# Kainmueller-Lab/PatchPerPix

Hardware: AMD Instinct MI355X
Metric: Mvoxels/sec assembled (vote_instances) (higher is better)
Workload: dtype f16 in, f32 accumulate

## Files before the change

include/ppp_mi355x.h:

```cpp
#ifndef PPP_MI355X_H
#define PPP_MI355X_H

#include <stddef.h>
#include <stdint.h>

#ifdef __cplusplus
extern "C" {
#endif

#define PPP_ABI_VERSION 5

enum ppp_error {
    PPP_OK = 0,
    PPP_ERR_INVALID_ARG = -1,
    PPP_ERR_NO_DEVICE = -2,
    PPP_ERR_HIP = -3,
    PPP_ERR_UNSUPPORTED = -4,
    PPP_ERR_WORKSPACE = -5
};

enum ppp_dtype { PPP_F32 = 0, PPP_F16 = 1, PPP_BF16 = 2 };

enum ppp_bg_rule { PPP_BG_INV_TH = 0, PPP_BG_HALF_TH = 1, PPP_BG_LESS_THAN_TH = 2 };
enum ppp_value_rule { PPP_VAL_COUNT = 0, PPP_VAL_PROB_PRODUCT = 1, PPP_VAL_NORM_PROB_PRODUCT = 2 };
// ... 210 lines not shown
                   const ppp_params *p, void *stream);

int64_t ppp_thin_shard_workspace_bytes(const ppp_params *p);
int ppp_thin_open(const uint8_t *d_mask, const int64_t *d_lin, const int32_t *d_index, int64_t n, int32_t *d_state,
                  int32_t *d_count, int32_t *d_cleared, void *d_work, const ppp_params *p, void *stream);
int ppp_thin_step(int32_t what, const uint32_t *d_bits, int32_t *d_state, int32_t *d_count, int32_t *d_cleared,
                  void *d_work, int32_t global_z, const ppp_params *p, void *stream);
int ppp_thin_alive(void *d_work, const ppp_params *p, void *stream, int32_t *alive);
int ppp_thin_close(uint8_t *d_mask, void *d_work, const ppp_params *p, void *stream);
int ppp_thin_zone(int32_t import, void *d_work, int32_t z_lo, int32_t z_hi, int32_t own_lo, int32_t own_hi,
                  int64_t *d_key, uint8_t *d_mask, uint8_t *d_clean, const ppp_params *p, void *stream);

int ppp_patch_pairs_count(const int32_t *d_sorted_zyx, int64_t n, int32_t max_ps_dist,
                          int64_t *d_counts, const ppp_params *p, void *stream);
int ppp_patch_pairs_fill(const int32_t *d_sorted_zyx, int64_t n, int32_t max_ps_dist,
                         const int64_t *d_offsets, int64_t n_pair_rows, int32_t include_single,
                         uint32_t *d_rows, const ppp_params *p, void *stream);
int ppp_patch_pairs_count_subset(const int32_t *d_sorted_zyx, int64_t n, int32_t max_ps_dist,
                                 const int64_t *d_subset, int64_t m, int64_t *d_counts,
                                 const ppp_params *p, void *stream);
int ppp_patch_pairs_fill_subset(const int32_t *d_sorted_zyx, int64_t n, int32_t max_ps_dist,
                                const int64_t *d_subset, int64_t m, const int64_t *d_local_offsets,
                                const int64_t *d_global_offsets, int64_t n_local_rows,
                                int64_t n_rows_total, int32_t include_single, uint32_t *d_rows,
                                int64_t *d_row_ids, const ppp_params *p, void *stream);
int ppp_patch_pairs_count_slices(const int32_t *d_sorted_zyx, int64_t n, int32_t max_ps_dist,
                                 int64_t *d_counts, const ppp_params *p, void *stream);
int ppp_patch_pairs_fill_slices(const int32_t *d_sorted_zyx, int64_t n, int32_t max_ps_dist,
                                const int64_t *d_offsets, int64_t n_pair_rows, int32_t include_single,
                                uint32_t *d_rows, const ppp_params *p, void *stream);
int ppp_patch_graph_slices(const void *d_pred, int pred_dtype, const float *d_cons,
                           const uint32_t *d_pairs, const uint32_t *d_order, uint64_t n_pairs,
                           float *d_aff, const ppp_params *p, void *stream);
int ppp_patch_graph_lcg_slices(const void *d_pred, int pred_dtype, const uint32_t *d_pairs,
                               const uint32_t *d_order, const int64_t *d_lcg_pos, int64_t n_lcg,
                               const int64_t *d_drop_off, uint64_t *d_drops, const ppp_params *p,
                               void *stream);
int ppp_patch_graph_by_patch_lcg_slices(const void *d_pred, int pred_dtype, const float *d_cons_vm,
                                        const uint32_t *d_pairs, const uint32_t *d_order,
                                        const int64_t *d_group_start, const int64_t *d_chunk_offsets,
                                        int32_t n_groups, int64_t n_blocks, int32_t chunk, float *d_aff,
                                        const int64_t *d_drop_off, const uint64_t *d_drops,
                                        const ppp_params *p, void *stream);
int ppp_thin_cover_slices(const uint8_t *d_mask, const uint32_t *d_bits, const int64_t *d_lin, int64_t n,
                          uint8_t *d_keep, void *d_work, const int64_t *h_slice_interior,
                          const ppp_params *p, void *stream, int32_t *rounds);
int ppp_label_slice_renumber(const uint32_t *d_nodes, uint64_t n_nodes, int32_t *d_labels,
                             int32_t *d_slice_min, int32_t *d_slice_max, const ppp_params *p, void *stream);

int ppp_pair_sort_keys(const uint32_t *d_rows, uint64_t n_rows, int64_t *d_keys,
                       const ppp_params *p, void *stream);
#define PPP_PAIR_KEY_FAR 0x7FFFFFFFFFFFFFFFll
int ppp_pair_group_keys(const uint32_t *d_rows, uint64_t n_rows, int64_t *d_keys,
                        const ppp_params *p, void *stream);

int64_t ppp_host_rank_order(const float *h_score, const uint8_t *h_foreground, const int32_t *vol,
                            const int32_t *patchshape, int64_t *out_lin);
int64_t ppp_host_cover_pass(uint8_t *h_mask_running, const uint8_t *h_overlap, const int32_t *vol,
                            const int32_t *patchshape, const int64_t *ranked_lin,
                            const float *ranked_score, const uint32_t *bits, int64_t n,
                            int32_t pix_th, double score_threshold, uint8_t *selected,
                            int64_t *remaining, int32_t *stopped);
int64_t ppp_host_cover_pass_marked(uint8_t *h_mask_running, const uint8_t *h_overlap, const int32_t *vol,
                                   const int32_t *patchshape, const int64_t *ranked_lin,
                                   const float *ranked_score, const uint32_t *bits, int64_t n,
                                   int32_t pix_th, double score_threshold, uint8_t *selected,
                                   int64_t *remaining, int32_t *stopped, uint8_t *h_marked);
int64_t ppp_host_thin_cover(const uint8_t *h_mask, const int32_t *vol, const int32_t *patchshape,
                            const int64_t *sel_lin, const uint32_t *bits, int64_t n,
                            uint8_t *keep);

int64_t ppp_host_skeletonize_3d(const uint8_t *h_mask, const int32_t *vol, uint8_t *h_out);
int64_t ppp_host_skel_rule_mismatches(uint32_t first, uint32_t count);
int64_t ppp_host_patch_pairs(const int32_t *sel_zyx, int64_t n, const int32_t *patchshape,
                             int32_t max_ps_dist, int32_t include_single, int32_t *sorted_zyx,
                             uint32_t *pairs);

int64_t ppp_host_mws(const uint32_t *pairs, const float *aff, int64_t n_rows, const int32_t *vol,
                     int32_t *out_nodes, int32_t *out_labels, int64_t cap, int64_t *n_labels);

int64_t ppp_host_mws_sorted(const int32_t *eu, const int32_t *ev, int64_t n_edges, int64_t n_nodes,
                            int32_t *labels);

int64_t ppp_host_pack_channels(int64_t n_labels, const int64_t *sizes, const uint64_t *pairs, int64_t n_pairs,
                               int64_t min_voxels, int32_t *chan_out, int32_t *n_channels_out);

int64_t ppp_rank_order_workspace_bytes(const ppp_params *p);
int ppp_rank_order(const float *d_score, const uint8_t *d_foreground, int64_t *d_lin,
                   float *d_rank_score, int64_t *count, void *d_work, const ppp_params *p,
                   void *stream);
int64_t ppp_mws_edges_workspace_bytes(int64_t n_rows, int64_t n_nodes, const ppp_params *p);
int ppp_mws_edges(const uint32_t *d_pairs, const float *d_aff, int64_t n_rows, const uint32_t *d_nodes,
                  int64_t n_nodes, int32_t *d_eu, int32_t *d_ev, int64_t *n_edges, void *d_work,
                  const ppp_params *p, void *stream);

int64_t ppp_post_compact_ids_workspace_bytes(int64_t n, uint32_t max_id);
int ppp_post_compact_ids(uint32_t *d_ids, int64_t n, uint32_t max_id, int64_t compsize, int32_t relabel,
                         uint32_t start, int64_t *n_kept, void *d_work, void *stream);
int64_t ppp_post_dilate_workspace_bytes(int32_t Z, int32_t Y, int32_t X);
int ppp_post_dilate(const uint32_t *d_in, uint32_t *d_out, int32_t Z, int32_t Y, int32_t X, int32_t *rounds,
                    void *d_work, void *stream);
int64_t ppp_post_clean_mask_workspace_bytes(int32_t Z, int32_t Y, int32_t X);
int ppp_post_clean_mask(const uint8_t *d_mask, uint8_t *d_out, int32_t Z, int32_t Y, int32_t X, uint32_t structure,
                        int64_t size, int64_t *n_found, int64_t *n_kept, void *d_work, void *stream);

int64_t ppp_post_edt_sq_workspace_bytes(int32_t Z, int32_t Y, int32_t X);
int ppp_post_edt_sq(const uint8_t *d_feature, uint32_t *d_out, int32_t Z, int32_t Y, int32_t X, uint32_t cap,
                    void *d_work, void *stream);
int64_t ppp_post_fg_filter_workspace_bytes(int32_t Z, int32_t Y, int32_t X);
int ppp_post_fg_filter(const uint8_t *d_mask, uint8_t *d_fg , uint32_t *d_inst ,
                       int32_t Z, int32_t Y, int32_t X, int64_t compsize, uint32_t min_d2,
                       int64_t *stats , void *d_work, void *stream);

int32_t ppp_eval_patch_thresholds_per_pass(void);
int32_t ppp_eval_patch_max_thresholds(void);
int64_t ppp_eval_patch_workspace_bytes(const int32_t *vol , int32_t tz);
int ppp_eval_patch(const void *d_pred, int pred_dtype, int32_t C, const int32_t *d_labels, int32_t L,
                   const int32_t *vol , const int32_t *patch , int32_t z0, int32_t tz,
                   const float *thresholds , int32_t T, int64_t *d_counts ,
                   int32_t *d_inter, int32_t *d_union , void *d_work, void *stream);

int64_t ppp_skeletonize_3d_workspace_bytes(int32_t Z, int32_t Y, int32_t X);
int ppp_skeletonize_3d(const uint8_t *d_mask, uint8_t *d_out, int32_t Z, int32_t Y, int32_t X,
                       int64_t *n_kept, int32_t *stats ,
                       void *d_work, void *stream);

int64_t ppp_skeletonize_labels_workspace_bytes(int32_t Z, int32_t Y, int32_t X);
int ppp_skeletonize_labels(const uint32_t *d_labels, uint32_t *d_out, int32_t Z, int32_t Y, int32_t X,
                           int64_t *n_kept, int32_t *stats ,
                           void *d_work, void *stream);

int32_t ppp_label_overlap_table_entries(void);
void ppp_label_overlap_last_stats(int64_t *stats );
uint32_t ppp_label_overlap_slot(uint32_t a, uint32_t b);
int64_t ppp_label_overlap_workspace_bytes(int32_t La, int32_t Lb, int32_t Z, int32_t Y, int32_t X);
int ppp_label_overlap(const uint32_t *d_a, int32_t La, const uint32_t *d_b, int32_t Lb,
                      int32_t Z, int32_t Y, int32_t X,
                      uint32_t *d_rows , int64_t *d_counts , int64_t cap,
                      int64_t *n_rows , void *d_work, void *stream);

int ppp_patch_mosaic(const void *d_pred, int pred_dtype, int32_t C, const uint8_t *d_selected, int32_t S,
                     void *d_out, int32_t tz, int32_t Y, int32_t X, const int32_t *patch , void *stream);

int ppp_gt_affs_dense_plan(int32_t B, int32_t L, const int32_t *vol , int32_t E, const int32_t *halo ,
                           const int32_t *box , int out_dtype, int32_t single, int32_t *plan );
int ppp_gt_affs_dense(const int32_t *d_labels, int32_t B, int32_t L, const int32_t *vol ,
                      const int32_t *d_nhood, int32_t E, const int32_t *halo ,
                      const int32_t *box , void *d_out, int out_dtype, int32_t single, void *stream);
int ppp_gt_affs_samples(const int32_t *d_labels, int32_t B, int32_t L, const int32_t *vol ,
                        const int32_t *d_samples , int64_t N, const int32_t *d_nhood, int32_t E,
                        const int32_t *ps , const int32_t *ctr , void *d_out, int out_dtype,
                        void *stream);

int64_t ppp_patch_loss_workspace_bytes(int32_t B, int32_t L, const int32_t *vol , int32_t E,
                                       const int32_t *halo , const int32_t *box ,
                                       int dtype, int64_t N );
int ppp_patch_loss_dense_fwd(const void *d_logits, int dtype, const int32_t *d_labels, int32_t B, int32_t L,
                             const int32_t *vol , const int32_t *d_nhood, int32_t E, const int32_t *halo ,
                             const int32_t *box , const float *d_weight , double num_channels,
                             float *d_loss , double *d_state , int64_t *d_counts ,
                             void *d_work, void *stream);
int ppp_patch_loss_dense_bwd(const void *d_logits, int dtype, const int32_t *d_labels, int32_t B, int32_t L,
                             const int32_t *vol , const int32_t *d_nhood, int32_t E, const int32_t *halo ,
                             const int32_t *box , const float *d_weight ,
                             const double *d_state , const float *d_grad_out , void *d_grad,
                             void *stream);
// ... 45 lines not shown
```

patchperpix_amd/backend.py:

```python
import ctypes
import os

import numpy as np

from . import build as _build

F32, F16, BF16 = 0, 1, 2
BG_INV_TH, BG_HALF_TH, BG_LESS_THAN_TH = 0, 1, 2
VAL_COUNT, VAL_PROB_PRODUCT, VAL_NORM_PROB_PRODUCT = 0, 1, 2
CONS_COMPACT, CONS_REFERENCE, CONS_VOXEL_MAJOR = 0, 1, 2
ABI_VERSION = 5
NONE_KEY = 0xFFFFFFFF
NONE_KEY64 = 1 << 62
PAIR_KEY_FAR = 0x7FFFFFFFFFFFFFFF


class Box(ctypes.Structure):
    _fields_ = [(n, ctypes.c_int32) for n in ("z0", "y0", "x0", "z1", "y1", "x1")]

    def shape(self):
        return (self.z1 - self.z0, self.y1 - self.y0, self.x1 - self.x0)


class Params(ctypes.Structure):
# ... 116 lines not shown
    "ppp_patch_graph_by_patch_bits": (ctypes.c_int, [ctypes.c_void_p, ctypes.c_int, ctypes.c_void_p,
                                                     ctypes.c_void_p, ctypes.c_void_p, ctypes.c_void_p,
                                                     ctypes.c_void_p, ctypes.c_int32, ctypes.c_int64,
                                                     ctypes.c_int32, ctypes.c_void_p, ctypes.c_void_p,
                                                     ctypes.c_void_p, ctypes.c_void_p, ctypes.c_int64,
                                                     ctypes.c_void_p, ctypes.c_int32,
                                                     ctypes.POINTER(Params), ctypes.c_void_p]),
    "ppp_label_workspace_bytes": (ctypes.c_size_t, [ctypes.POINTER(Params)]),
    "ppp_label_components": (ctypes.c_int, [ctypes.c_void_p, ctypes.c_void_p, ctypes.c_uint64,
                                            ctypes.c_void_p, ctypes.c_uint64, ctypes.c_void_p,
                                            ctypes.c_void_p, ctypes.POINTER(Params),
                                            ctypes.c_void_p]),
    "ppp_label_begin": (ctypes.c_int, [ctypes.c_void_p, ctypes.c_uint64, ctypes.c_void_p,
                                       ctypes.POINTER(Params), ctypes.c_void_p]),
    "ppp_label_add": (ctypes.c_int, [ctypes.c_void_p, ctypes.c_void_p, ctypes.c_void_p,
                                     ctypes.c_int64, ctypes.c_uint64, ctypes.c_void_p,
                                     ctypes.POINTER(Params), ctypes.c_void_p]),
    "ppp_label_union_edges": (ctypes.c_int, [ctypes.c_void_p, ctypes.c_void_p, ctypes.c_uint64,
                                             ctypes.c_void_p, ctypes.POINTER(Params),
                                             ctypes.c_void_p]),
    "ppp_label_finish": (ctypes.c_int, [ctypes.c_void_p, ctypes.c_uint64, ctypes.c_void_p,
                                        ctypes.c_void_p, ctypes.POINTER(Params), ctypes.c_void_p]),
    "ppp_patch_pairs_count_subset": (ctypes.c_int, [ctypes.c_void_p, ctypes.c_int64, ctypes.c_int32,
                                                    ctypes.c_void_p, ctypes.c_int64, ctypes.c_void_p,
                                                    ctypes.POINTER(Params), ctypes.c_void_p]),
    "ppp_patch_pairs_fill_subset": (ctypes.c_int, [ctypes.c_void_p, ctypes.c_int64, ctypes.c_int32,
                                                   ctypes.c_void_p, ctypes.c_int64, ctypes.c_void_p,
                                                   ctypes.c_void_p, ctypes.c_int64, ctypes.c_int64,
                                                   ctypes.c_int32, ctypes.c_void_p, ctypes.c_void_p,
                                                   ctypes.POINTER(Params), ctypes.c_void_p]),
    "ppp_patch_pairs_count": (ctypes.c_int, [ctypes.c_void_p, ctypes.c_int64, ctypes.c_int32,
                                             ctypes.c_void_p, ctypes.POINTER(Params),
                                             ctypes.c_void_p]),
    "ppp_patch_pairs_fill": (ctypes.c_int, [ctypes.c_void_p, ctypes.c_int64, ctypes.c_int32,
                                            ctypes.c_void_p, ctypes.c_int64, ctypes.c_int32,
                                            ctypes.c_void_p, ctypes.POINTER(Params),
                                            ctypes.c_void_p]),
    "ppp_pair_sort_keys": (ctypes.c_int, [ctypes.c_void_p, ctypes.c_uint64, ctypes.c_void_p,
                                          ctypes.POINTER(Params), ctypes.c_void_p]),
    "ppp_paint_instances": (ctypes.c_int, [ctypes.c_void_p, ctypes.c_int, ctypes.c_void_p,
                                           ctypes.c_void_p, ctypes.c_uint64, ctypes.c_void_p,
                                           ctypes.POINTER(Params), ctypes.c_void_p]),
    "ppp_cons_to_reference": (ctypes.c_int, [ctypes.c_void_p, ctypes.c_void_p,
                                             ctypes.POINTER(Params), ctypes.c_void_p]),
    "ppp_cons_to_voxel_major": (ctypes.c_int, [ctypes.c_void_p, ctypes.c_void_p,
                                               ctypes.POINTER(Params), ctypes.c_void_p]),
    "ppp_patch_bits": (ctypes.c_int, [ctypes.c_void_p, ctypes.c_int, ctypes.c_void_p,
                                      ctypes.c_uint64, ctypes.c_double, ctypes.c_void_p,
                                      ctypes.POINTER(Params), ctypes.c_void_p]),
    "ppp_patch_bits_volume": (ctypes.c_int, [ctypes.c_void_p, ctypes.c_int, ctypes.c_double,
                                             ctypes.c_void_p, ctypes.POINTER(Params), ctypes.c_void_p]),
    "ppp_pair_group_keys": (ctypes.c_int, [ctypes.c_void_p, ctypes.c_uint64, ctypes.c_void_p,
                                           ctypes.POINTER(Params), ctypes.c_void_p]),
    "ppp_patch_graph_by_patch_chunk": (ctypes.c_int32, [ctypes.POINTER(Params)]),
    "ppp_cover_workspace_bytes": (ctypes.c_int64, [ctypes.c_int64, ctypes.POINTER(Params)]),
    "ppp_cover_pass": (ctypes.c_int, [ctypes.c_void_p, ctypes.c_void_p, ctypes.c_void_p,
                                      ctypes.c_int64, ctypes.c_int32, ctypes.c_void_p,
                                      ctypes.c_void_p, ctypes.c_void_p, ctypes.POINTER(Params),
                                      ctypes.c_void_p, ctypes.POINTER(ctypes.c_int32)]),
    "ppp_cover_pass_voxel_bits": (ctypes.c_int, [ctypes.c_void_p, ctypes.c_void_p, ctypes.c_int64,
                                                 ctypes.c_void_p, ctypes.c_int64, ctypes.c_int32,
                                                 ctypes.c_void_p, ctypes.c_void_p, ctypes.c_void_p,
                                                 ctypes.POINTER(Params), ctypes.c_void_p,
                                                 ctypes.POINTER(ctypes.c_int32)]),
    "ppp_cover_pass_marked": (ctypes.c_int, [ctypes.c_void_p, ctypes.c_void_p, ctypes.c_void_p,
                                             ctypes.c_int64, ctypes.c_int32, ctypes.c_void_p,
                                             ctypes.c_void_p, ctypes.c_void_p, ctypes.c_void_p,
                                             ctypes.POINTER(Params), ctypes.c_void_p,
                                             ctypes.POINTER(ctypes.c_int32)]),
    "ppp_cover_pass_marked_voxel_bits": (ctypes.c_int, [ctypes.c_void_p, ctypes.c_void_p, ctypes.c_int64,
                                                        ctypes.c_void_p, ctypes.c_int64, ctypes.c_int32,
                                                        ctypes.c_void_p, ctypes.c_void_p, ctypes.c_void_p,
                                                        ctypes.c_void_p, ctypes.POINTER(Params),
                                                        ctypes.c_void_p, ctypes.POINTER(ctypes.c_int32)]),
    "ppp_cover_mark_bits_bytes": (ctypes.c_int64, [ctypes.POINTER(Params)]),
    "ppp_cover_marks_from_selected": (ctypes.c_int, [ctypes.c_void_p, ctypes.c_void_p, ctypes.c_int64,
                                                     ctypes.c_void_p, ctypes.POINTER(Params),
                                                     ctypes.c_void_p]),
    "ppp_mask_dilate_workspace_bytes": (ctypes.c_int64, [ctypes.POINTER(Params)]),
    "ppp_mask_dilate": (ctypes.c_int, [ctypes.c_void_p, ctypes.c_void_p, ctypes.c_int32, ctypes.c_int32,
                                       ctypes.c_void_p, ctypes.POINTER(Params), ctypes.c_void_p]),
    "ppp_host_mws_sorted": (ctypes.c_int64, [ctypes.c_void_p, ctypes.c_void_p, ctypes.c_int64,
                                             ctypes.c_int64, ctypes.c_void_p]),
    "ppp_rank_order_workspace_bytes": (ctypes.c_int64, [ctypes.POINTER(Params)]),
    "ppp_rank_order": (ctypes.c_int, [ctypes.c_void_p, ctypes.c_void_p, ctypes.c_void_p,
                                      ctypes.c_void_p, ctypes.POINTER(ctypes.c_int64),
                                      ctypes.c_void_p, ctypes.POINTER(Params), ctypes.c_void_p]),
    "ppp_mws_edges_workspace_bytes": (ctypes.c_int64, [ctypes.c_int64, ctypes.c_int64,
                                                       ctypes.POINTER(Params)]),
    "ppp_mws_edges": (ctypes.c_int, [ctypes.c_void_p, ctypes.c_void_p, ctypes.c_int64,
                                     ctypes.c_void_p, ctypes.c_int64, ctypes.c_void_p,
                                     ctypes.c_void_p, ctypes.POINTER(ctypes.c_int64),
                                     ctypes.c_void_p, ctypes.POINTER(Params), ctypes.c_void_p]),
    "ppp_thin_workspace_bytes": (ctypes.c_int64, [ctypes.c_int64, ctypes.POINTER(Params)]),
    "ppp_thin_cover": (ctypes.c_int, [ctypes.c_void_p, ctypes.c_void_p, ctypes.c_void_p,
                                      ctypes.c_int64, ctypes.c_void_p, ctypes.c_void_p,
                                      ctypes.POINTER(Params), ctypes.c_void_p,
                                      ctypes.POINTER(ctypes.c_int32)]),
    "ppp_cover_open": (ctypes.c_int, [ctypes.c_void_p, ctypes.c_void_p, ctypes.c_void_p,
                                      ctypes.c_int64, ctypes.c_void_p, ctypes.c_void_p,
                                      ctypes.c_void_p, ctypes.POINTER(Params), ctypes.c_void_p]),
    "ppp_cover_step": (ctypes.c_int, [ctypes.c_int32, ctypes.c_void_p, ctypes.c_int32,
                                      ctypes.c_void_p, ctypes.c_void_p, ctypes.c_void_p,
                                      ctypes.c_int32, ctypes.POINTER(Params), ctypes.c_void_p]),
    "ppp_cover_alive": (ctypes.c_int, [ctypes.c_void_p, ctypes.POINTER(Params), ctypes.c_void_p,
                                       ctypes.POINTER(ctypes.c_int32)]),
    "ppp_cover_close": (ctypes.c_int, [ctypes.c_void_p, ctypes.c_void_p, ctypes.POINTER(Params),
                                       ctypes.c_void_p]),
    "ppp_cover_zone": (ctypes.c_int, [ctypes.c_int32, ctypes.c_void_p, ctypes.c_int32,
                                      ctypes.c_int32, ctypes.c_int32, ctypes.c_int32,
                                      ctypes.c_void_p, ctypes.c_void_p, ctypes.c_void_p,
                                      ctypes.POINTER(Params), ctypes.c_void_p]),
    "ppp_thin_shard_workspace_bytes": (ctypes.c_int64, [ctypes.POINTER(Params)]),
    "ppp_thin_open": (ctypes.c_int, [ctypes.c_void_p, ctypes.c_void_p, ctypes.c_void_p, ctypes.c_int64,
                                     ctypes.c_void_p, ctypes.c_void_p, ctypes.c_void_p, ctypes.c_void_p,
                                     ctypes.POINTER(Params), ctypes.c_void_p]),
    "ppp_thin_step": (ctypes.c_int, [ctypes.c_int32, ctypes.c_void_p, ctypes.c_void_p, ctypes.c_void_p,
                                     ctypes.c_void_p, ctypes.c_void_p, ctypes.c_int32, ctypes.POINTER(Params),
                                     ctypes.c_void_p]),
    "ppp_thin_alive": (ctypes.c_int, [ctypes.c_void_p, ctypes.POINTER(Params), ctypes.c_void_p,
                                      ctypes.POINTER(ctypes.c_int32)]),
    "ppp_thin_close": (ctypes.c_int, [ctypes.c_void_p, ctypes.c_void_p, ctypes.POINTER(Params), ctypes.c_void_p]),
    "ppp_thin_zone": (ctypes.c_int, [ctypes.c_int32, ctypes.c_void_p, ctypes.c_int32, ctypes.c_int32,
                                     ctypes.c_int32, ctypes.c_int32, ctypes.c_void_p, ctypes.c_void_p,
                                     ctypes.c_void_p, ctypes.POINTER(Params), ctypes.c_void_p]),
    "ppp_synth_pred": (ctypes.c_int, [ctypes.c_void_p, ctypes.c_void_p, ctypes.c_int,
                                      ctypes.c_uint32, ctypes.c_float, ctypes.c_float,
                                      ctypes.c_float, ctypes.c_uint64, ctypes.POINTER(Params),
                                      ctypes.c_void_p]),
    "ppp_synth_pred_box": (ctypes.c_int, [ctypes.c_void_p, ctypes.c_void_p, ctypes.c_void_p, ctypes.c_int,
                                          ctypes.c_uint32, ctypes.c_float, ctypes.c_float, ctypes.c_float,
                                          ctypes.c_void_p, ctypes.POINTER(Params), ctypes.c_void_p]),
    "ppp_decode_tail": (ctypes.c_int, [ctypes.c_void_p, ctypes.c_int64, ctypes.c_int32, ctypes.c_int32,
                                       ctypes.c_void_p, ctypes.c_float, ctypes.c_void_p, ctypes.c_float,
                                       ctypes.c_void_p, ctypes.c_float, ctypes.c_void_p, ctypes.c_void_p,
                                       ctypes.c_int, ctypes.POINTER(Params), ctypes.c_void_p]),
    "ppp_decode_tail_rows": (ctypes.c_int, [ctypes.c_void_p, ctypes.c_int64, ctypes.c_int32, ctypes.c_int32,
                                            ctypes.c_void_p, ctypes.c_float, ctypes.c_void_p, ctypes.c_float,
                                            ctypes.c_void_p, ctypes.c_float, ctypes.c_void_p, ctypes.c_void_p,
                                            ctypes.c_int, ctypes.c_int32, ctypes.c_void_p]),
    "ppp_rows_index_bytes": (ctypes.c_int64, [ctypes.c_int32, ctypes.c_int32, ctypes.c_int32]),
    "ppp_rows_index_build": (ctypes.c_int, [ctypes.c_void_p, ctypes.c_int32, ctypes.c_int32, ctypes.c_int32,
                                            ctypes.c_void_p, ctypes.POINTER(ctypes.c_int64), ctypes.c_void_p]),
    "ppp_rows_expand": (ctypes.c_int, [ctypes.c_void_p, ctypes.c_int, ctypes.c_int32, ctypes.c_void_p,
                                       ctypes.c_int32, ctypes.c_int32, ctypes.c_int32, ctypes.POINTER(Box),
                                       ctypes.c_void_p, ctypes.c_void_p]),
    "ppp_rows_compact": (ctypes.c_int, [ctypes.c_void_p, ctypes.c_int, ctypes.c_int32, ctypes.POINTER(Box),
                                        ctypes.c_void_p, ctypes.c_int32, ctypes.c_int32, ctypes.c_int32,
                                        ctypes.c_void_p, ctypes.c_void_p]),
    "ppp_host_mws":(ctypes.c_int64, [ctypes.c_void_p, ctypes.c_void_p, ctypes.c_int64,
                                      ctypes.c_void_p, ctypes.c_void_p, ctypes.c_void_p,
                                      ctypes.c_int64, ctypes.POINTER(ctypes.c_int64)]),
    "ppp_host_rank_order": (ctypes.c_int64, [ctypes.c_void_p, ctypes.c_void_p, ctypes.c_void_p,
                                             ctypes.c_void_p, ctypes.c_void_p]),
    "ppp_host_cover_pass": (ctypes.c_int64, [ctypes.c_void_p, ctypes.c_void_p, ctypes.c_void_p,
                                             ctypes.c_void_p, ctypes.c_void_p, ctypes.c_void_p,
                                             ctypes.c_void_p, ctypes.c_int64, ctypes.c_int32,
                                             ctypes.c_double, ctypes.c_void_p,
                                             ctypes.POINTER(ctypes.c_int64),
                                             ctypes.POINTER(ctypes.c_int32)]),
    "ppp_host_cover_pass_marked": (ctypes.c_int64, [ctypes.c_void_p, ctypes.c_void_p, ctypes.c_void_p,
                                                    ctypes.c_void_p, ctypes.c_void_p, ctypes.c_void_p,
                                                    ctypes.c_void_p, ctypes.c_int64, ctypes.c_int32,
                                                    ctypes.c_double, ctypes.c_void_p,
                                                    ctypes.POINTER(ctypes.c_int64),
                                                    ctypes.POINTER(ctypes.c_int32), ctypes.c_void_p]),
# ... 2031 lines not shown
```

patchperpix_amd/csrc/ppp_host_mws.cpp:

```cpp
#include <stdint.h>

#include <algorithm>
#include <unordered_map>
#include <unordered_set>
#include <vector>

#include "../../include/ppp_mi355x.h"

namespace {

struct Edge {
    int32_t a, b;
    float w;
    int8_t attractive;
};

struct Dsu {
    std::vector<int32_t> parent;
    int32_t find(int32_t x) {
        while (parent[x] != x) {
            parent[x] = parent[parent[x]];
            x = parent[x];
        }
        return x;
    }
};

struct KeySet {
    static constexpr uint64_t EMPTY = ~0ull, TOMB = ~0ull - 1;
    std::vector<uint64_t> slot;
    size_t used = 0, live = 0;
    explicit KeySet(size_t cap = 1024) : slot(cap, EMPTY) {}
    static size_t hash(uint64_t k) {
        k ^= k >> 33; k *= 0xff51afd7ed558ccdull; k ^= k >> 33; k *= 0xc4ceb9fe1a85ec53ull; k ^= k >> 33;
        return (size_t)k;
    }
    void grow() {
        std::vector<uint64_t> old;
        old.swap(slot);
        slot.assign(live * 4 + 1024 > old.size() ? old.size() * 2 : old.size(), EMPTY);
        used = live = 0;
        for (uint64_t k : old)
            if (k != EMPTY && k != TOMB) insert(k);
    }
    bool contains(uint64_t k) const {
        const size_t m = slot.size() - 1;
        for (size_t i = hash(k) & m;; i = (i + 1) & m) {
            if (slot[i] == k) return true;
            if (slot[i] == EMPTY) return false;
        }
    }
    bool insert(uint64_t k) {
        if ((used + 1) * 2 > slot.size()) grow();
        const size_t m = slot.size() - 1;
        size_t tomb = (size_t)-1;
        for (size_t i = hash(k) & m;; i = (i + 1) & m) {
            if (slot[i] == k) return false;
            if (slot[i] == TOMB && tomb == (size_t)-1) tomb = i;
            if (slot[i] == EMPTY) {
                if (tomb != (size_t)-1) { slot[tomb] = k; }
                else { slot[i] = k; ++used; }
                ++live;
                return true;
            }
        }
    }
    void erase(uint64_t k) {
        const size_t m = slot.size() - 1;
        for (size_t i = hash(k) & m;; i = (i + 1) & m) {
            if (slot[i] == k) { slot[i] = TOMB; --live; return; }
            if (slot[i] == EMPTY) return;
        }
    }
};

void watershed(const int32_t *eu, const int32_t *ev, int64_t n_edges, int32_t N, int32_t *label,
               int64_t *issued) {
    Dsu dsu;
    dsu.parent.resize((size_t)N);
    for (int32_t i = 0; i < N; ++i) dsu.parent[i] = i;
    std::vector<int32_t> cc_of_root((size_t)N, 0);
    std::vector<std::vector<int32_t>> nbrs((size_t)N);
    KeySet mutex(1 << 16);
    std::vector<uint8_t> alive((size_t)N + 2, 0);
    int32_t max_alive = 0;
    std::vector<int32_t> created;
    std::vector<uint8_t> ever;
    ever.assign((size_t)N + 2, 0);
    auto key = [](int32_t a, int32_t b) -> uint64_t {
        const uint32_t lo = (uint32_t)std::min(a, b), hi = (uint32_t)std::max(a, b);
        return ((uint64_t)lo << 32) | hi;
    };
    auto has_mutex = [&](int32_t r0, int32_t r1) { return mutex.contains(key(r0, r1)); };
    std::vector<int32_t> n_nbrs((size_t)N, 0);
    auto unite = [&](int32_t ra, int32_t rb) -> int32_t {
        int32_t keep = ra, drop = rb;
        if (n_nbrs[keep] < n_nbrs[drop]) std::swap(keep, drop);
        if (n_nbrs[drop]) {
            std::vector<int32_t> &kl = nbrs[keep], &dl = nbrs[drop];
            for (int32_t x : dl) {
                const int32_t p = dsu.find(x);
                if (p == keep || p == drop) continue;
                mutex.erase(key(drop, p));
                if (mutex.insert(key(keep, p))) kl.push_back(p);
            }
            mutex.erase(key(keep, drop));
            std::vector<int32_t>().swap(dl);
            n_nbrs[keep] = (int32_t)kl.size();
            n_nbrs[drop] = 0;
        }
        dsu.parent[drop] = keep;
        return keep;
    };
    constexpr int64_t AHEAD = 24;
    for (int64_t i = 0; i < n_edges; ++i) {
        if (i + AHEAD < n_edges) {
            const int32_t pa = eu[i + AHEAD], pb = ev[i + AHEAD] & 0x7FFFFFFF;
            __builtin_prefetch(&dsu.parent[pa]);
            __builtin_prefetch(&dsu.parent[pb]);
        }
        const int32_t a = eu[i], b = ev[i] & 0x7FFFFFFF;
        const int32_t r0 = dsu.find(a), r1 = dsu.find(b);
        if (ev[i] < 0) {
            const int32_t c0 = cc_of_root[r0], c1 = cc_of_root[r1];
            if (c0 == 0 && c1 == 0) {
                while (max_alive > 0 && !alive[(size_t)max_alive]) --max_alive;
                const int32_t id = max_alive + 1;
                const int32_t r = r0 != r1 ? unite(r0, r1) : r0;
                cc_of_root[r] = id;
                alive[(size_t)id] = 1;
                max_alive = id;
                if (!ever[(size_t)id]) { ever[(size_t)id] = 1; created.push_back(id); }
            } else if (c0 == 0 || c1 == 0) {
                if (!has_mutex(r0, r1)) {
                    const int32_t id = c0 == 0 ? c1 : c0;
                    cc_of_root[unite(r0, r1)] = id;
                }
            } else if (c0 != c1) {
                if (!has_mutex(r0, r1)) {
                    const int32_t keep = std::min(c0, c1), drop = std::max(c0, c1);
                    cc_of_root[unite(r0, r1)] = keep;
                    alive[(size_t)drop] = 0;
                }
            }
        } else if (r0 != r1) {
            if (mutex.insert(key(r0, r1))) {
                nbrs[r0].push_back(r1);
                nbrs[r1].push_back(r0);
                ++n_nbrs[r0];
                ++n_nbrs[r1];
            }
        }
    }
    std::vector<int32_t> label_of_id((size_t)N + 2, 0);
    for (size_t i = 0; i < created.size(); ++i) label_of_id[(size_t)created[i]] = (int32_t)i + 1;
    for (int32_t n = 0; n < N; ++n) label[n] = label_of_id[(size_t)cc_of_root[dsu.find(n)]];
    *issued = (int64_t)created.size();
}

}

extern "C" {

int64_t ppp_host_mws_sorted(const int32_t *eu, const int32_t *ev, int64_t n_edges, int64_t n_nodes,
                            int32_t *labels) {
    int64_t issued = 0;
    if (n_nodes <= 0) return 0;
    watershed(eu, ev, n_edges, (int32_t)n_nodes, labels, &issued);
    return issued;
}

int64_t ppp_host_mws(const uint32_t *pairs, const float *aff, int64_t n_rows, const int32_t *vol,
                     int32_t *out_nodes, int32_t *out_labels, int64_t cap, int64_t *n_labels) {
    const int64_t Y = vol[1], X = vol[2];
    auto lin = [&](const uint32_t *c) { return ((int64_t)c[0] * Y + c[1]) * X + c[2]; };

    const int64_t V = (int64_t)vol[0] * Y * X;
    const bool direct = V <= (1ll << 28);
    std::vector<int32_t> table(direct ? (size_t)V : 0, -1);
    std::unordered_map<int64_t, int32_t> node_id;
    std::vector<int64_t> node_key;
    struct Row { int32_t u, v; float a; };
    std::vector<Row> rows;
    rows.reserve((size_t)n_rows);
    for (int64_t i = 0; i < n_rows; ++i) {
        if (aff[i] == 0.0f) continue;
        int32_t id[2];
        for (int s = 0; s < 2; ++s) {
            const int64_t k = lin(pairs + i * 6 + 3 * s);
            if (direct) {
                if (k < 0 || k >= V) return -2;
                if (table[k] < 0) {
                    table[k] = (int32_t)node_key.size();
                    node_key.push_back(k);
                }
                id[s] = table[k];
            } else {
                auto it = node_id.find(k);
                if (it == node_id.end()) {
                    it = node_id.emplace(k, (int32_t)node_key.size()).first;
                    node_key.push_back(k);
                }
                id[s] = it->second;
            }
        }
        rows.push_back({id[0], id[1], aff[i]});
    }
    std::vector<int32_t>().swap(table);
    const int32_t N = (int32_t)node_key.size();
    if (N > cap) return -1;
    {
        std::vector<uint64_t> key(rows.size());
        for (size_t i = 0; i < rows.size(); ++i) {
            const uint32_t lo = (uint32_t)std::min(rows[i].u, rows[i].v), hi = (uint32_t)std::max(rows[i].u, rows[i].v);
            key[i] = ((uint64_t)lo << 32) | hi;
        }
        std::vector<uint64_t> sorted(key);
        std::sort(sorted.begin(), sorted.end());
        if (std::adjacent_find(sorted.begin(), sorted.end()) != sorted.end()) {
            std::unordered_map<uint64_t, size_t> first;
            std::vector<Row> uniq;
            for (size_t i = 0; i < rows.size(); ++i) {
                auto it = first.find(key[i]);
                if (it == first.end()) {
                    first.emplace(key[i], uniq.size());
                    uniq.push_back(rows[i]);
                } else {
                    uniq[it->second].a = rows[i].a;
                }
            }
            rows.swap(uniq);
        }
    }
    std::vector<int64_t> start((size_t)N + 1, 0);
    for (const Row &r : rows) {
        ++start[r.u + 1];
        if (r.u != r.v) ++start[r.v + 1];
    }
    for (int32_t n = 0; n < N; ++n) start[n + 1] += start[n];
    std::vector<int32_t> nbr((size_t)start[N]);
    std::vector<float> nbr_a((size_t)start[N]);
    {
        std::vector<int64_t> fill(start.begin(), start.end() - 1);
        for (const Row &r : rows) {
            nbr[fill[r.u]] = r.v; nbr_a[fill[r.u]++] = r.a;
            if (r.u != r.v) { nbr[fill[r.v]] = r.u; nbr_a[fill[r.v]++] = r.a; }
        }
    }
    std::vector<Edge> edges;
    edges.reserve(rows.size());
    for (int32_t n = 0; n < N; ++n)
        for (int64_t j = start[n]; j < start[n + 1]; ++j)
            if (nbr[j] >= n) {
                const float a = nbr_a[j];
                edges.push_back(a > 0 ? Edge{n, nbr[j], a, 1} : Edge{n, nbr[j], -a, -1});
            }
    std::vector<int32_t>().swap(nbr);
    std::vector<float>().swap(nbr_a);
    std::vector<Row>().swap(rows);
    std::stable_sort(edges.begin(), edges.end(), [](const Edge &x, const Edge &y) { return x.w > y.w; });

    std::vector<int32_t> eu(edges.size()), ev(edges.size());
    for (size_t i = 0; i < edges.size(); ++i) {
        eu[i] = edges[i].a;
        ev[i] = edges[i].b | (edges[i].attractive == 1 ? (int32_t)0x80000000 : 0);
    }
    std::vector<Edge>().swap(edges);
    std::vector<int32_t> label((size_t)N);
    int64_t issued = 0;
    watershed(eu.data(), ev.data(), (int64_t)eu.size(), N, label.data(), &issued);

    for (int32_t n = 0; n < N; ++n) {
        const int64_t k = node_key[n];
        out_nodes[3 * (int64_t)n + 0] = (int32_t)(k / (Y * X));
        out_nodes[3 * (int64_t)n + 1] = (int32_t)((k / X) % Y);
        out_nodes[3 * (int64_t)n + 2] = (int32_t)(k % X);
        out_labels[n] = label[(size_t)n];
    }
    if (n_labels) *n_labels = issued;
    return N;
}

}
```

Before: 17.16.

## Prune settled edges in parallel between sequential mutex watershed blocks

Splits the sorted-edge mutex watershed into growing blocks. After each block the union-find is compressed, and a thread pool classifies the remaining edges as already settled (same component or already mutex-separated), then compacts out the settled ones so the sequential pass visits fewer edges. This trades extra parallel scans and array copies for a shorter serial union-find loop, and it only applies when there are at least 200k edges. Stats and per-edge classification entry points are added for diagnostics.

```diff
diff --git a/include/ppp_mi355x.h b/include/ppp_mi355x.h
--- a/include/ppp_mi355x.h
+++ b/include/ppp_mi355x.h
@@ -316,6 +316,13 @@
 int64_t ppp_host_mws_sorted(const int32_t *eu, const int32_t *ev, int64_t n_edges, int64_t n_nodes,
                             int32_t *labels);
 
+#define PPP_MWS_N_STATS 8
+int64_t ppp_host_mws_sorted_stats(const int32_t *eu, const int32_t *ev, int64_t n_edges, int64_t n_nodes,
+                                  int32_t *labels, int64_t *stats);
+
+int64_t ppp_host_mws_sorted_classes(const int32_t *eu, const int32_t *ev, int64_t n_edges, int64_t n_nodes,
+                                    int32_t *labels, uint8_t *cls);
+
 int64_t ppp_host_pack_channels(int64_t n_labels, const int64_t *sizes, const uint64_t *pairs, int64_t n_pairs,
                                int64_t min_voxels, int32_t *chan_out, int32_t *n_channels_out);
 
diff --git a/patchperpix_amd/backend.py b/patchperpix_amd/backend.py
--- a/patchperpix_amd/backend.py
+++ b/patchperpix_amd/backend.py
@@ -222,6 +222,10 @@
                                        ctypes.c_void_p, ctypes.POINTER(Params), ctypes.c_void_p]),
     "ppp_host_mws_sorted": (ctypes.c_int64, [ctypes.c_void_p, ctypes.c_void_p, ctypes.c_int64,
                                              ctypes.c_int64, ctypes.c_void_p]),
+    "ppp_host_mws_sorted_stats": (ctypes.c_int64, [ctypes.c_void_p, ctypes.c_void_p, ctypes.c_int64,
+                                                   ctypes.c_int64, ctypes.c_void_p, ctypes.c_void_p]),
+    "ppp_host_mws_sorted_classes": (ctypes.c_int64, [ctypes.c_void_p, ctypes.c_void_p, ctypes.c_int64,
+                                                     ctypes.c_int64, ctypes.c_void_p, ctypes.c_void_p]),
     "ppp_rank_order_workspace_bytes": (ctypes.c_int64, [ctypes.POINTER(Params)]),
     "ppp_rank_order": (ctypes.c_int, [ctypes.c_void_p, ctypes.c_void_p, ctypes.c_void_p,
                                       ctypes.c_void_p, ctypes.POINTER(ctypes.c_int64),
diff --git a/patchperpix_amd/csrc/ppp_host_mws.cpp b/patchperpix_amd/csrc/ppp_host_mws.cpp
--- a/patchperpix_amd/csrc/ppp_host_mws.cpp
+++ b/patchperpix_amd/csrc/ppp_host_mws.cpp
@@ -1,6 +1,13 @@
 #include <stdint.h>
+#include <stdlib.h>
 
 #include <algorithm>
+#include <condition_variable>
+#include <functional>
+#include <memory>
+#include <mutex>
+#include <system_error>
+#include <thread>
 #include <unordered_map>
 #include <unordered_set>
 #include <vector>
@@ -74,26 +81,114 @@
     }
 };
 
-void watershed(const int32_t *eu, const int32_t *ev, int64_t n_edges, int32_t N, int32_t *label,
-               int64_t *issued) {
+class Pool {
+    int n_ = 1;
+    std::vector<std::thread> th_;
+    std::mutex m_;
+    std::condition_variable go_, done_;
+    uint64_t gen_ = 0;
+    int pending_ = 0;
+    bool stop_ = false;
+    const std::function<void(int)> *job_ = nullptr;
+    void worker(int t) {
+        uint64_t seen = 0;
+        std::unique_lock<std::mutex> l(m_);
+        for (;;) {
+            go_.wait(l, [&] { return gen_ != seen; });
+            seen = gen_;
+            if (stop_) return;
+            const std::function<void(int)> *f = job_;
+            l.unlock();
+            (*f)(t);
+            l.lock();
+            if (--pending_ == 0) done_.notify_one();
+        }
+    }
+
+public:
+    explicit Pool(int n) {
+        th_.reserve((size_t)std::max(n, 1));
+        try {
+            for (int t = 1; t < n; ++t) {
+                th_.emplace_back([this, t] { worker(t); });
+                ++n_;
+            }
+        } catch (const std::system_error &) {}
+    }
+    ~Pool() {
+        {
+            std::lock_guard<std::mutex> l(m_);
+            stop_ = true;
+            ++gen_;
+        }
+        go_.notify_all();
+        for (std::thread &t : th_) t.join();
+    }
+    int size() const { return n_; }
+    void run(const std::function<void(int)> &f) {
+        {
+            std::lock_guard<std::mutex> l(m_);
+            job_ = &f;
+            pending_ = n_ - 1;
+            ++gen_;
+        }
+        go_.notify_all();
+        f(0);
+        std::unique_lock<std::mutex> l(m_);
+        done_.wait(l, [&] { return pending_ == 0; });
+    }
+};
+
+int prune_threads() {
+    int n = 16;
+    const unsigned hw = std::thread::hardware_concurrency();
+    if (hw > 0 && (int)hw < n) n = (int)hw;
+    if (const char *s = getenv("OMP_NUM_THREADS")) {
+        const long v = strtol(s, nullptr, 10);
+        if (v >= 1 && v < n) n = (int)v;
+    }
+    return n;
+}
+
+int64_t env_i64(const char *name, int64_t fallback) {
+    const char *s = getenv(name);
+    if (!s || !*s) return fallback;
+    char *end = nullptr;
+    const long long v = strtoll(s, &end, 10);
+    return end == s || v < 0 ? fallback : (int64_t)v;
+}
+
+enum { ST_BLOCKS = 0, ST_RULE1, ST_RULE2, ST_RULE3, ST_RULE4, ST_VISITED, ST_THREADS, ST_PRUNES, ST_N };
+static_assert(ST_N == PPP_MWS_N_STATS, "stats layout");
+enum { CL_A_NEW = 0, CL_A_JOIN, CL_A_MERGE, CL_A_SAME, CL_A_REFUSED, CL_R_SAME, CL_R_KNOWN, CL_R_INSERT };
+
+constexpr int64_t PRUNE_FIRST_SHARE = 8, PRUNE_GROWTH = 4;
+constexpr int64_t PRUNE_MIN_EDGES = 200000;
+
+struct Mws {
+    int32_t N;
     Dsu dsu;
-    dsu.parent.resize((size_t)N);
-    for (int32_t i = 0; i < N; ++i) dsu.parent[i] = i;
-    std::vector<int32_t> cc_of_root((size_t)N, 0);
-    std::vector<std::vector<int32_t>> nbrs((size_t)N);
-    KeySet mutex(1 << 16);
-    std::vector<uint8_t> alive((size_t)N + 2, 0);
+    std::vector<int32_t> cc_of_root;
+    std::vector<std::vector<int32_t>> nbrs;
+    std::vector<int32_t> n_nbrs;
+    KeySet mutex;
+    std::vector<uint8_t> alive;
     int32_t max_alive = 0;
     std::vector<int32_t> created;
     std::vector<uint8_t> ever;
-    ever.assign((size_t)N + 2, 0);
-    auto key = [](int32_t a, int32_t b) -> uint64_t {
+
+    explicit Mws(int32_t n)
+        : N(n), cc_of_root((size_t)n, 0), nbrs((size_t)n), n_nbrs((size_t)n, 0), mutex(1 << 16),
+          alive((size_t)n + 2, 0), ever((size_t)n + 2, 0) {
+        dsu.parent.resize((size_t)n);
+        for (int32_t i = 0; i < n; ++i) dsu.parent[i] = i;
+    }
+    static uint64_t key(int32_t a, int32_t b) {
         const uint32_t lo = (uint32_t)std::min(a, b), hi = (uint32_t)std::max(a, b);
         return ((uint64_t)lo << 32) | hi;
-    };
-    auto has_mutex = [&](int32_t r0, int32_t r1) { return mutex.contains(key(r0, r1)); };
-    std::vector<int32_t> n_nbrs((size_t)N, 0);
-    auto unite = [&](int32_t ra, int32_t rb) -> int32_t {
+    }
+    bool has_mutex(int32_t r0, int32_t r1) const { return mutex.contains(key(r0, r1)); }
+    int32_t unite(int32_t ra, int32_t rb) {
         int32_t keep = ra, drop = rb;
         if (n_nbrs[keep] < n_nbrs[drop]) std::swap(keep, drop);
         if (n_nbrs[drop]) {
@@ -111,51 +206,148 @@
         }
         dsu.parent[drop] = keep;
         return keep;
-    };
-    constexpr int64_t AHEAD = 24;
-    for (int64_t i = 0; i < n_edges; ++i) {
-        if (i + AHEAD < n_edges) {
-            const int32_t pa = eu[i + AHEAD], pb = ev[i + AHEAD] & 0x7FFFFFFF;
-            __builtin_prefetch(&dsu.parent[pa]);
-            __builtin_prefetch(&dsu.parent[pb]);
-        }
-        const int32_t a = eu[i], b = ev[i] & 0x7FFFFFFF;
-        const int32_t r0 = dsu.find(a), r1 = dsu.find(b);
-        if (ev[i] < 0) {
-            const int32_t c0 = cc_of_root[r0], c1 = cc_of_root[r1];
-            if (c0 == 0 && c1 == 0) {
-                while (max_alive > 0 && !alive[(size_t)max_alive]) --max_alive;
-                const int32_t id = max_alive + 1;
-                const int32_t r = r0 != r1 ? unite(r0, r1) : r0;
-                cc_of_root[r] = id;
-                alive[(size_t)id] = 1;
-                max_alive = id;
-                if (!ever[(size_t)id]) { ever[(size_t)id] = 1; created.push_back(id); }
-            } else if (c0 == 0 || c1 == 0) {
-                if (!has_mutex(r0, r1)) {
-                    const int32_t id = c0 == 0 ? c1 : c0;
-                    cc_of_root[unite(r0, r1)] = id;
-                }
-            } else if (c0 != c1) {
-                if (!has_mutex(r0, r1)) {
-                    const int32_t keep = std::min(c0, c1), drop = std::max(c0, c1);
-                    cc_of_root[unite(r0, r1)] = keep;
-                    alive[(size_t)drop] = 0;
-                }
-            }
-        } else if (r0 != r1) {
-            if (mutex.insert(key(r0, r1))) {
-                nbrs[r0].push_back(r1);
-                nbrs[r1].push_back(r0);
-                ++n_nbrs[r0];
-                ++n_nbrs[r1];
-            }
-        }
-    }
-    std::vector<int32_t> label_of_id((size_t)N + 2, 0);
-    for (size_t i = 0; i < created.size(); ++i) label_of_id[(size_t)created[i]] = (int32_t)i + 1;
-    for (int32_t n = 0; n < N; ++n) label[n] = label_of_id[(size_t)cc_of_root[dsu.find(n)]];
-    *issued = (int64_t)created.size();
+    }
+
+    template <bool TRACE>
+    void visit(const int32_t *eu, const int32_t *ev, int64_t n_edges, uint8_t *cls) {
+        constexpr int64_t AHEAD = 24;
+        for (int64_t i = 0; i < n_edges; ++i) {
+            if (i + AHEAD < n_edges) {
+                const int32_t pa = eu[i + AHEAD], pb = ev[i + AHEAD] & 0x7FFFFFFF;
+                __builtin_prefetch(&dsu.parent[pa]);
+                __builtin_prefetch(&dsu.parent[pb]);
+            }
+            const int32_t a = eu[i], b = ev[i] & 0x7FFFFFFF;
+            const int32_t r0 = dsu.find(a), r1 = dsu.find(b);
+            if (ev[i] < 0) {
+                const int32_t c0 = cc_of_root[r0], c1 = cc_of_root[r1];
+                if (TRACE) cls[i] = CL_A_SAME;
+                if (c0 == 0 && c1 == 0) {
+                    while (max_alive > 0 && !alive[(size_t)max_alive]) --max_alive;
+                    const int32_t id = max_alive + 1;
+                    const int32_t r = r0 != r1 ? unite(r0, r1) : r0;
+                    cc_of_root[r] = id;
+                    alive[(size_t)id] = 1;
+                    max_alive = id;
+                    if (!ever[(size_t)id]) { ever[(size_t)id] = 1; created.push_back(id); }
+                    if (TRACE) cls[i] = CL_A_NEW;
+                } else if (c0 == 0 || c1 == 0) {
+                    if (TRACE) cls[i] = CL_A_REFUSED;
+                    if (!has_mutex(r0, r1)) {
+                        const int32_t id = c0 == 0 ? c1 : c0;
+                        cc_of_root[unite(r0, r1)] = id;
+                        if (TRACE) cls[i] = CL_A_JOIN;
+                    }
+                } else if (c0 != c1) {
+                    if (TRACE) cls[i] = CL_A_REFUSED;
+                    if (!has_mutex(r0, r1)) {
+                        const int32_t keep = std::min(c0, c1), drop = std::max(c0, c1);
+                        cc_of_root[unite(r0, r1)] = keep;
+                        alive[(size_t)drop] = 0;
+                        if (TRACE) cls[i] = CL_A_MERGE;
+                    }
+                }
+            } else if (r0 != r1) {
+                if (TRACE) cls[i] = CL_R_KNOWN;
+                if (mutex.insert(key(r0, r1))) {
+                    nbrs[r0].push_back(r1);
+                    nbrs[r1].push_back(r0);
+                    ++n_nbrs[r0];
+                    ++n_nbrs[r1];
+                    if (TRACE) cls[i] = CL_R_INSERT;
+                }
+            } else if (TRACE) {
+                cls[i] = CL_R_SAME;
+            }
+        }
+    }
+
+    int settled(int32_t a, int32_t evb) const {
+        const int32_t r0 = dsu.parent[a], r1 = dsu.parent[evb & 0x7FFFFFFF];
+        if (evb < 0) {
+            if (r0 == r1) return cc_of_root[r0] != 0 ? 2 : 0;
+            return (cc_of_root[r0] != 0 || cc_of_root[r1] != 0) && has_mutex(r0, r1) ? 4 : 0;
+        }
+        if (r0 == r1) return 1;
+        return has_mutex(r0, r1) ? 3 : 0;
+    }
+    void compress() {
+        for (int32_t x = 0; x < N; ++x) dsu.parent[x] = dsu.find(x);
+    }
+
+    void labels(int32_t *label, int64_t *issued) {
+        std::vector<int32_t> label_of_id((size_t)N + 2, 0);
+        for (size_t i = 0; i < created.size(); ++i) label_of_id[(size_t)created[i]] = (int32_t)i + 1;
+        for (int32_t n = 0; n < N; ++n) label[n] = label_of_id[(size_t)cc_of_root[dsu.find(n)]];
+        *issued = (int64_t)created.size();
+    }
+};
+
+struct alignas(64) Slice {
+    int64_t dropped[5] = {0, 0, 0, 0, 0};
+    int64_t kept = 0, at = 0;
+};
+
+void watershed(const int32_t *eu, const int32_t *ev, int64_t n_edges, int32_t N, int32_t *label,
+               int64_t *issued, int64_t *stats) {
+    int64_t st[ST_N] = {0};
+    Mws w(N);
+    const int64_t min_len = env_i64("PPP_MWS_PRUNE_MIN", PRUNE_MIN_EDGES);
+    const int64_t fixed_block = env_i64("PPP_MWS_PRUNE_BLOCK", 0);
+    if (env_i64("PPP_MWS_PRUNE", 1) == 0 || n_edges < min_len || n_edges == 0) {
+        w.visit<false>(eu, ev, n_edges, nullptr);
+        st[ST_VISITED] = n_edges;
+    } else {
+        Pool pool(prune_threads());
+        const int T = pool.size();
+        st[ST_THREADS] = T;
+        std::vector<Slice> part((size_t)T);
+        std::unique_ptr<int32_t[]> su, sv;
+        std::unique_ptr<uint8_t[]> rule;
+        const int32_t *cu = eu, *cv = ev;
+        int64_t left = n_edges;
+        int64_t block = fixed_block > 0 ? fixed_block : std::max<int64_t>(n_edges / PRUNE_FIRST_SHARE, 1);
+        for (;;) {
+            const int64_t b = std::min(block, left);
+            w.visit<false>(cu, cv, b, nullptr);
+            ++st[ST_BLOCKS];
+            st[ST_VISITED] += b;
+            cu += b; cv += b; left -= b;
+            if (left == 0) break;
+            w.compress();
+            if (!rule) rule.reset(new uint8_t[(size_t)left]);
+            const int64_t per = (left + T - 1) / T;
+            pool.run([&](int t) {
+                Slice &s = part[(size_t)t];
+                s.kept = 0;
+                const int64_t lo = std::min(left, per * t), hi = std::min(left, lo + per);
+                for (int64_t i = lo; i < hi; ++i) {
+                    const int r = w.settled(cu[i], cv[i]);
+                    rule[(size_t)i] = (uint8_t)r;
+                    ++s.dropped[r];
+                    s.kept += r == 0;
+                }
+            });
+            int64_t kept = 0;
+            for (Slice &s : part) { s.at = kept; kept += s.kept; }
+            std::unique_ptr<int32_t[]> nu(new int32_t[(size_t)kept]), nv(new int32_t[(size_t)kept]);
+            pool.run([&](int t) {
+                int64_t at = part[(size_t)t].at;
+                const int64_t lo = std::min(left, per * t), hi = std::min(left, lo + per);
+                for (int64_t i = lo; i < hi; ++i)
+                    if (rule[(size_t)i] == 0) { nu[(size_t)at] = cu[i]; nv[(size_t)at] = cv[i]; ++at; }
+            });
+            su.swap(nu); sv.swap(nv);
+            cu = su.get(); cv = sv.get(); left = kept;
+            ++st[ST_PRUNES];
+            if (left == 0) break;
+            if (fixed_block <= 0) block *= PRUNE_GROWTH;
+        }
+        for (const Slice &s : part)
+            for (int r = 1; r <= 4; ++r) st[ST_RULE1 + r - 1] += s.dropped[r];
+    }
+    w.labels(label, issued);
+    if (stats) std::copy(st, st + ST_N, stats);
 }
 
 }
@@ -164,9 +356,25 @@
 
 int64_t ppp_host_mws_sorted(const int32_t *eu, const int32_t *ev, int64_t n_edges, int64_t n_nodes,
                             int32_t *labels) {
+    return ppp_host_mws_sorted_stats(eu, ev, n_edges, n_nodes, labels, nullptr);
+}
+
+int64_t ppp_host_mws_sorted_stats(const int32_t *eu, const int32_t *ev, int64_t n_edges, int64_t n_nodes,
+                                  int32_t *labels, int64_t *stats) {
+    int64_t issued = 0;
+    if (stats) std::fill(stats, stats + PPP_MWS_N_STATS, 0);
+    if (n_nodes <= 0) return 0;
+    watershed(eu, ev, n_edges, (int32_t)n_nodes, labels, &issued, stats);
+    return issued;
+}
+
+int64_t ppp_host_mws_sorted_classes(const int32_t *eu, const int32_t *ev, int64_t n_edges, int64_t n_nodes,
+                                    int32_t *labels, uint8_t *cls) {
     int64_t issued = 0;
     if (n_nodes <= 0) return 0;
-    watershed(eu, ev, n_edges, (int32_t)n_nodes, labels, &issued);
+    Mws w((int32_t)n_nodes);
+    w.visit<true>(eu, ev, n_edges, cls);
+    w.labels(labels, &issued);
     return issued;
 }
 
@@ -268,7 +476,7 @@
     std::vector<Edge>().swap(edges);
     std::vector<int32_t> label((size_t)N);
     int64_t issued = 0;
-    watershed(eu.data(), ev.data(), (int64_t)eu.size(), N, label.data(), &issued);
+    watershed(eu.data(), ev.data(), (int64_t)eu.size(), N, label.data(), &issued, nullptr);
 
     for (int32_t n = 0; n < N; ++n) {
         const int64_t k = node_key[n];
```

Measured after the change: 17.97, median of 6. 4.7% higher.
